# Anttwo/MACARONS

Measured on AMD Instinct MI355X. Metric: candidate-camera coverage-gain evals/sec (100k pts, 200 cams), higher is better.
Workload: dtype f32; 1 GPU; scorer: B=1 cloud x N=100000 points x C=200 cameras per GPU (BASELINE headline 100k pts / 200 cams), inputs resident in HBM; points=100000, cams_per_gpu=200, parallelism=camera-shard x1, streams=2

## Files before the change

macarons_amd/csrc/networks.hip:

```cpp
#include "nn_kernels.h"
#include "net_layout.h"
#include <cstdlib>
#include <algorithm>
#include <map>
#include <mutex>
#include <utility>

namespace mcr {

#ifdef MCR_DEV_LOCAL_PCT8
void launch_local_pct8(hipStream_t s, const float* offs, float* feat, int64_t ld_feat, int64_t S, const float* blob);
#define MCR_VARIANT8_OK(v) ((v) == 8)
#else
#define MCR_VARIANT8_OK(v) false
#endif
static int g_default_variant = []() {
    const char* e = getenv("MCR_LOCAL_PCT_VARIANT");
    const int v = e ? atoi(e) : 6;
    return (v == 1 || v == 5 || v == 6) ? v : 6;
}();
static thread_local int t_next_variant = 0;
static thread_local int t_variant = 0;
static thread_local int t_scope_depth = 0;
struct VariantScope {
// ... 454 lines not shown
    if (planes) {
        launch_linear_smallk_planes(s, {pts, 4}, l1.w, l1.b, ACT_GELU, h128, T, VIS_F, 4, 128);
        const float* b2 = w.b_l2p;
        const WPlanes W2 = weight_planes(s, w.p_l2, WSPLIT_INV, l2, VIS_F, VIS_F, VIS_F, ff, 128, 128, &b2);
        launch_linear3p(s, h128, W2, {b2, ACT_NONE}, {x, VIS_E}, T, 128, 128, np);
    } else {
        launch_linear(s, {pts, 4}, {l1.w, 4}, {l1.b, ACT_GELU}, {h, VIS_F}, T, VIS_F, 4, N);
        launch_linear(s, {h, VIS_F}, {l2.w, VIS_F}, {l2.b, ACT_NONE}, {x, VIS_E}, T, VIS_F, VIS_F, N);
    }
    launch_colmax_broadcast(s, x, VIS_E, x + VIS_F, VIS_E, B, (int)N, VIS_F, lengths, pts, 4, 4, x + 2 * VIS_F);
    for (int e = 0; e < 3; ++e) run_encoder(s, w.enc[e], x, h, qkv, ff, B, (int)N, VIS_E, 4, lengths);
    if (planes) {
        launch_layernorm_planes(s, {x, VIS_E}, w.ng, w.nb, hP.keep(np), T, VIS_E);
        _Float16* q = reinterpret_cast<_Float16*>(qkv);
        const WPlanes W1 = weight_planes(s, w.p_fc1, WSPLIT_INV, fc1, VIS_E, 192, VIS_E, q);
        const WPlanes W2 = weight_planes(s, w.p_fc2, WSPLIT_INV, fc2, VIS_E, 128, VIS_E, q + 2 * 192 * VIS_E);
        const WPlanes W3 = weight_planes(s, w.p_fc3, WSPLIT_INV, fc3, 128, 64, 128, q + 2 * (192 + 128) * VIS_E);
        const Planes fP = planes_over(ff, T, VIS_E);
        launch_linear3p(s, hP, W1, {fc1.b, ACT_GELU}, fP, T, 192, VIS_E, np);
        launch_split_to_planes(s, {view_harmonics, 64}, fP.cols(192).keep(np), T, 64);
        launch_linear3p(s, fP, W2, {fc2.b, ACT_GELU}, h128, T, 128, VIS_E, np);
        launch_linear3p(s, h128, W3, {fc3.b, ACT_NONE}, {out, 64}, T, 64, 128, np);
    } else {
        launch_layernorm(s, x, VIS_E, w.ng, w.nb, h, VIS_E, T, VIS_E);
        launch_linear(s, {h, VIS_E}, {fc1.w, VIS_E}, {fc1.b, ACT_GELU}, {ff, VIS_E}, T, 192, VIS_E, seq_route(N));
        launch_copy2d(s, view_harmonics, 64, ff + 192, VIS_E, T, 64);
        launch_linear(s, {ff, VIS_E}, {fc2.w, VIS_E}, {fc2.b, ACT_GELU}, {h, 128}, T, 128, VIS_E, seq_route(N));
        launch_linear(s, {h, 128}, {fc3.w, 128}, {fc3.b, ACT_NONE}, {out, 64}, T, 64, 128, N);
    }
    MCR_LAUNCH_CHECK("mcr_scone_vis_forward");
    return 0;
}

constexpr int OCC_CHUNK = 16384;
constexpr int FEAT = 1344;
constexpr size_t OCC_WS_SLACK = 8192 + 2 * 1024, OCC_RAGGED_WS_SLACK = 8192 + 1024;

struct OccHead {
    float *feat, *h1, *h2, *gfeat, *gbias;
    void* wplanes;
    HeadScratch planes() const { return HeadScratch{reinterpret_cast<_Float16*>(feat), reinterpret_cast<_Float16*>(h1), h2, wplanes}; }
};
static OccHead carve_occ_head(Arena& a, int64_t T, int64_t G) {
    OccHead w;
    w.feat = a.f(T * FEAT);
    w.h1 = a.f(T * 512);
    w.h2 = a.f(T * 256);
    w.gfeat = a.f(G * 512);
    w.gbias = a.f(G * 512);
    w.wplanes = a.bytes(linear3h_planes_bytes(512, 1344));
    return w;
}

struct OccSide { hipStream_t s = nullptr; hipEvent_t fork = nullptr, join = nullptr; };
static OccSide* occ_side(hipStream_t caller, int slot = 0) {
    static const bool on = []() { const char* e = getenv("MCR_OCC_OVERLAP"); return !(e && e[0] == '0'); }();
    if (!on) return nullptr;
    static std::mutex mu;
    static std::map<std::pair<std::pair<int, int>, hipStream_t>, OccSide> table;
    int dev = 0;
    if (hipGetDevice(&dev) != hipSuccess) return nullptr;
    std::lock_guard<std::mutex> lock(mu);
    OccSide& x = table[std::make_pair(std::make_pair(dev, slot), caller)];
    if (!x.s) {
        if (hipStreamCreateWithFlags(&x.s, hipStreamNonBlocking) != hipSuccess || hipEventCreateWithFlags(&x.fork, hipEventDisableTiming) != hipSuccess ||
            hipEventCreateWithFlags(&x.join, hipEventDisableTiming) != hipSuccess) {
            x.s = nullptr;
            return nullptr;
        }
    }
    return &x;
}
static hipStream_t fork_side(hipStream_t s, OccSide*& side) {
    if (side && hipEventRecord(side->fork, s) == hipSuccess && hipStreamWaitEvent(side->s, side->fork, 0) == hipSuccess) return side->s;
    side = nullptr;
    return s;
}
struct SideJoin {
    OccSide* side; hipStream_t s; bool recorded = false, joined = false;
    ~SideJoin() {
        if (!side || joined) return;
        if (!recorded) (void)hipEventRecord(side->join, side->s);
        (void)hipStreamWaitEvent(s, side->join, 0);
    }
};

static void run_global(hipStream_t gs, const OccW& w, const float* pc_global, int64_t G, int64_t Lg, const int* lens, const EncScratch& glob,
                       const OccHead& hd) {
    run_pct(gs, w.global, pc_global, hd.gfeat, 512, G, (int)Lg, 256, glob, lens);
    launch_linear(gs, {hd.gfeat, 512}, {w.lin1.w, 1856}, {nullptr, ACT_NONE}, {hd.gbias, 512}, G, 512, 512, 1);
}

static void head_linear(hipStream_t s, int which, Rows X, const LinW& lin, int64_t ldw, RowsOut Y, int64_t M, int N, int K, RowBias rb,
                        const void* const* head_planes, const float* head_inv_scales, void* wplanes) {
    const int variant = g_local_pct_variant;
    const int64_t ANY_M = (int64_t)1 << 40;
    const Rows W{lin.w, ldw};
    const Epilogue e{lin.b, ACT_GELU, {}, rb};
    if ((variant == 6 || variant == 7) && linear3h_applicable(X.p, X.ld, W.p, W.ld, ANY_M, N, K))
        launch_linear3h(s, X, head_weight_planes(s, which, lin, ldw, N, K, head_planes, head_inv_scales, wplanes), e, Y, M, N, K);
    else if (variant == 5 && linear3_applicable(X.p, X.ld, W.p, W.ld, ANY_M, N, K))
        launch_linear3(s, X, W, e, Y, M, N, K);
    else
        launch_linear(s, X, W, e, Y, M, N, K, 1);
}

static int run_occ_head(const char* who, hipStream_t s, const OccW& w, const float* x, const float* view_harmonics, int64_t T, const OccHead& hd,
                        int64_t rows_per_group, const int* row_group, const void* const* head_planes, const float* head_inv_scales, bool planes,
                        bool x_done, OccSide* side, SideJoin& side_join, int* range_flag, float* out) {
    bool join_failed = false;
    auto join = [&]() {
        if (side) {
            side_join.joined = true;
            join_failed = hipStreamWaitEvent(s, side->join, 0) != hipSuccess;
        }
    };
    if (planes)
        run_head_planes(s, x, view_harmonics, T, w.xe1, w.xe2, w.xe3, w.lin1, w.lin2, w.lin3, hd.gbias, rows_per_group, row_group, head_planes,
                        head_inv_scales, hd.planes(), out, join, x_done);
    else {
        launch_linear(s, {x, 3}, {w.xe1.w, 3}, {w.xe1.b, ACT_GELU}, {hd.h2, 128}, T, 128, 3, 1);
        head_linear(s, 0, {hd.h2, 128}, w.xe2, 128, {hd.h1, 256}, T, 256, 128, {}, head_planes, head_inv_scales, hd.wplanes);
        head_linear(s, 1, {hd.h1, 256}, w.xe3, 256, {hd.feat + 768, FEAT}, T, 512, 256, {}, head_planes, head_inv_scales, hd.wplanes);
        launch_copy2d(s, view_harmonics, 64, hd.feat + 1280, FEAT, T, 64);
        join();
        MCR_REQUIRE(!join_failed, "%s: side stream (join)", who);
        head_linear(s, 2, {hd.feat, FEAT}, {w.lin1.w + 512, w.lin1.b}, 1856, {hd.h1, 512}, T, 512, FEAT, {hd.gbias, rows_per_group, row_group},
                    head_planes, head_inv_scales, hd.wplanes);
        head_linear(s, 3, {hd.h1, 512}, w.lin2, 512, {hd.h2, 256}, T, 256, 512, {}, head_planes, head_inv_scales, hd.wplanes);
        launch_linear(s, {hd.h2, 256}, {w.lin3.w, 256}, {w.lin3.b, ACT_GELU}, {out, 1}, T, 1, 256, 1);
    }
    MCR_REQUIRE(!join_failed, "%s: side stream (join)", who);
    if (range_flag) launch_nonfinite_flag(s, out, T, range_flag);
    MCR_LAUNCH_CHECK(who);
    return 0;
}

struct OccLocal { float* offs; EncScratch pct; };
static OccLocal carve_occ_local(Arena& a, int64_t rows, bool layer_by_layer) {
    OccLocal w{};
    w.offs = a.f(rows * 16 * 3);
    if (layer_by_layer) w.pct = carve_enc(a, rows * 16, PCT_E);
    return w;
}
struct OccScratch {
    OccHead head;
    char *knn_q, *knn_c, *knn_park;
    size_t knn_c_bytes;
    EncScratch glob;
    Arena scratch;
};
static OccScratch carve_occ(Arena& a, int64_t B, int64_t Q, int64_t Lg) {
    OccScratch w;
    w.head = carve_occ_head(a, B * Q, B);
    w.knn_c_bytes = knn_grid_cloud_bytes(B, 16384);
    w.knn_q = (char*)a.bytes(knn_grid_query_bytes(B, Q));
    w.knn_c = (char*)a.bytes(3 * w.knn_c_bytes);
    w.knn_park = (char*)a.bytes(knn_grid_park_bytes());
    w.glob = carve_enc(a, B * Lg, PCT_E);
    w.scratch = a.rest();
    return w;
}
size_t mcr_scone_occ_workspace_bytes(int64_t B, int64_t Q, int64_t Lg) {
    const size_t local = std::max({measure(carve_occ_local, B * Q, false), measure(carve_occ_local, Q, false),
                                   measure(carve_occ_local, std::min<int64_t>(Q, OCC_CHUNK), true)});
    return measure(carve_occ, B, Q, Lg) + local + OCC_WS_SLACK;
}

int mcr_knn_points(const float* X, const float* pc, int64_t* idx, float* dists, float* pts, int64_t B, int64_t Q, int64_t M,
                   int k, int subtract_query, void* stream);

int mcr_scone_occ_forward_phase(const float* pc_global, int64_t Lg, const float* const* pc_scale, const int64_t* M_scale,
                                const float* x, const float* view_harmonics, float* out, int64_t B, int64_t Q,
                                const float* const* weights, int n_weights, const float* const* local_blobs,
                                const void* const* head_planes, const float* head_inv_scales, int* range_flag, void* workspace,
                                size_t workspace_bytes, int phase, void* stream) {
    const char* who = "mcr_scone_occ_forward";
    VariantScope variant_scope_;
    MCR_REQUIRE(phase >= 0 && phase <= 2, "mcr_scone_occ_forward: phase must be 0, 1 or 2");
    const bool early = phase != 2, late = phase != 1;
    MCR_REQUIRE(pc_scale && M_scale && x && weights && (!late || (pc_global && view_harmonics && out)), "mcr_scone_occ_forward: null pointer");
    MCR_REQUIRE(!head_planes || head_inv_scales, "mcr_scone_occ_forward: head_planes need head_inv_scales");
    if (check_table(who, OCC_TABLE, weights, n_weights, n_weights)) return 1;
    MCR_REQUIRE(B > 0 && Q > 0 && Lg > 0 && B <= 65535, "mcr_scone_occ_forward: bad problem size");
    MCR_REQUIRE(workspace && workspace_bytes >= mcr_scone_occ_workspace_bytes(B, Q, Lg), "mcr_scone_occ_forward: workspace too small");
    for (int i = 0; i < 3; ++i)
        MCR_REQUIRE((pc_scale[i] || (!late && i > 0)) && M_scale[i] >= 16, "mcr_scone_occ_forward: scale %d has %ld points (< k = 16)", i,
                    (long)M_scale[i]);
    hipStream_t s = (hipStream_t)stream;
    const OccW w = read_occ_table(weights, n_weights);
    Arena arena{(char*)workspace, workspace_bytes};
    const OccScratch ws = carve_occ(arena, B, Q, Lg);
    MCR_REQUIRE(arena.ok(), "mcr_scone_occ_forward: workspace overflow (global)");
    const OccHead& hd = ws.head;
    float* feat = hd.feat;

    OccSide* side = late ? occ_side(s) : nullptr;
    const hipStream_t gs = fork_side(s, side);
    SideJoin side_join{side, s};
    const bool fused_all = local_blobs && local_blobs[0] && local_blobs[1] && local_blobs[2];
    const int64_t qc = fused_all ? Q : std::min<int64_t>(Q, OCC_CHUNK);
    const bool planes = fused_all && fp16_planes_variant();
    const int64_t Tall = B * Q;
    const Planes featP = planes_over(hd.feat, Tall, FEAT);
    OccSide* xside = planes ? occ_side(s, 1) : nullptr;
    struct XJoin {
        OccSide* side; hipStream_t s; bool armed;
        bool wait() { if (!armed) return true; armed = false; return hipStreamWaitEvent(s, side->join, 0) == hipSuccess; }
        ~XJoin() { (void)wait(); }
    } x_join{xside, s, false};
    if (xside && early) {
        MCR_REQUIRE(hipEventRecord(xside->fork, s) == hipSuccess && hipStreamWaitEvent(xside->s, xside->fork, 0) == hipSuccess,
                    "mcr_scone_occ_forward: side stream (x embedding fork)");
        run_x_embedding_planes(xside->s, x, nullptr, B * Q, w.xe1, w.xe2, w.xe3, head_planes, head_inv_scales, hd.planes());
        MCR_REQUIRE(hipEventRecord(xside->join, xside->s) == hipSuccess, "mcr_scone_occ_forward: side stream (x embedding record)");
        x_join.armed = true;
    }
    if (late) {
        run_global(gs, w, pc_global, B, Lg, nullptr, ws.glob, hd);
        if (xside)
            launch_split_to_planes(gs, {view_harmonics, 64}, featP.cols(1280).keep(matrix_planes()), B * Q, 64);
    }
    if (side) {
        MCR_REQUIRE(hipEventRecord(side->join, side->s) == hipSuccess, "mcr_scone_occ_forward: side stream (record)");
        side_join.recorded = true;
    }
    const int* knn_qperm = nullptr;
    KnnGridCloud knn_clouds[3]{};
    int knn_slot[3] = {-1, -1, -1};
    if (qc == Q) {
        const float* g_pc[3]; int64_t g_M[3]; void* g_ws[3];
        int n_grid = 0;
        for (int sc = 0; sc < 3; ++sc)
            if (knn_grid_applicable(M_scale[sc], 16)) {
                g_pc[n_grid] = pc_scale[sc]; g_M[n_grid] = M_scale[sc]; g_ws[n_grid] = ws.knn_c + n_grid * ws.knn_c_bytes;
                knn_slot[sc] = n_grid++;
            }
        if (n_grid) {
            if (phase == 0) {
                knn_qperm = knn_grid_order_queries(s, x, B, Q, ws.knn_q, ws.knn_park);
                knn_grid_build_clouds(s, n_grid, g_pc, g_M, B, g_ws, knn_clouds);
            } else {
                const int first = early ? 0 : (knn_slot[0] >= 0 ? 1 : 0), count = early ? (knn_slot[0] >= 0 ? 1 : 0) : n_grid - first;
                OccSide* bside = early && count > 0 ? occ_side(s) : nullptr;
                const hipStream_t bs = fork_side(s, bside);
                knn_grid_build_clouds(bs, count, g_pc + first, g_M + first, B, g_ws + first, knn_clouds + first);
                const bool recorded = !bside || hipEventRecord(bside->join, bside->s) == hipSuccess;
                knn_qperm = knn_grid_order_queries(s, x, B, Q, ws.knn_q, ws.knn_park, early);
                const bool joined = !bside || hipStreamWaitEvent(s, bside->join, 0) == hipSuccess;
                MCR_REQUIRE(recorded && joined, "mcr_scone_occ_forward: side stream (cloud build)");
            }
            MCR_LAUNCH_CHECK("knn grid preparation");
        }
    }
    for (int sc = 0; sc < 3; ++sc) {
        if (sc == 0 ? !early : !late) continue;
        const bool grid_knn = knn_slot[sc] >= 0;
        const KnnGridCloud knn_cloud = grid_knn ? knn_clouds[knn_slot[sc]] : KnnGridCloud{};
        const bool fused = planes || (local_blobs && local_blobs[sc]);
        if (B > 1 && qc == Q && fused) {
            Arena a = ws.scratch;
            float* offs = carve_occ_local(a, Tall, false).offs;
            MCR_REQUIRE(a.ok(), "mcr_scone_occ_forward: workspace overflow (kNN)");
            if (grid_knn) {
                launch_knn16_grid(s, x, pc_scale[sc], M_scale[sc], knn_qperm, knn_cloud, 0, B, Q, nullptr, nullptr, offs, true, ws.knn_park, sc);
                MCR_LAUNCH_CHECK("knn_grid_kernel");
            } else if (int e = mcr_knn_points(x, pc_scale[sc], nullptr, nullptr, offs, B, Q, M_scale[sc], 16, 1, stream))
                return e;
            if (planes) run_local_pct(s, offs, nullptr, FEAT, Tall, local_blobs[sc], featP.cols(sc * 256));
            else run_local_pct(s, offs, feat + sc * 256, FEAT, Tall, local_blobs[sc]);
            continue;
        }
        for (int64_t q0 = 0; q0 < Q; q0 += qc) {
            const int64_t nq = std::min<int64_t>(qc, Q - q0);
            for (int64_t b = 0; b < B; ++b) {
                Arena a = ws.scratch;
                const OccLocal loc = carve_occ_local(a, nq, !fused);
                MCR_REQUIRE(a.ok(), fused ? "mcr_scone_occ_forward: workspace overflow (kNN)" : "mcr_scone_occ_forward: workspace overflow (local)");
                float* offs = loc.offs;
// ... 113 lines not shown
```

macarons_amd/nbv.py:

```python

import torch

from . import dist as mdist
from .utility import scone_utils as su


class ViewStateGrid:

    def __init__(self, device, degree=8, n_elev=7, n_azim=14):
        self.n_elev, self.n_azim = n_elev, n_azim
        self.base_harmonics, self.h_polar, self.h_azim = su.get_all_harmonics_under_degree(degree, n_elev, n_azim, device)


_side_streams = {}


def _harmonics_beside(scone_occ, pc, Xl, harmonics_of):
    dev = Xl.device
    main = torch.cuda.current_stream(dev)
    fork = torch.cuda.Event()
    fork.record(main)
    begun = scone_occ.forward_begin(pc, Xl)
    if begun is None:
        return begun, harmonics_of(Xl)
    side = _side_streams.get((dev.index, main.cuda_stream))
    if side is None:
        side = _side_streams[(dev.index, main.cuda_stream)] = torch.cuda.Stream(device=dev)
    side.wait_event(fork)
    with torch.cuda.stream(side):
        vh = harmonics_of(Xl)
    main.wait_stream(side)
    vh.record_stream(main)
    return begun, vh


def _guarded(impl, scone_occ, range_guard, group, draws, device, scone_vis=None):
    from . import ops
    capturing = torch.cuda.is_current_stream_capturing()
    prev = scone_occ.range_guard
    guard = range_guard and prev != "off" and ops.current_variant() in (6, 7)
    scone_occ.range_guard = "defer" if (guard or prev != "off") else "off"
    vis_prev = None
    if scone_vis is not None and hasattr(scone_vis, "range_guard"):
        vis_prev = (scone_vis.range_guard, scone_vis._range_flag)
        scone_vis.range_guard = scone_occ.range_guard
    try:
        flagged = scone_occ.range_guard != "off" and ops.current_variant() in (6, 7)
        scone_occ.clear_range_flag(device if flagged else None)
        if vis_prev is not None:
            scone_vis._range_flag = scone_occ.range_flag()
        kw = draws() if (guard and not capturing) else {}
        out = impl(**kw)
        flag = scone_occ.range_flag() if ops.current_variant() in (6, 7) else None
        out["range_flag"] = flag
        if guard and not capturing:
            xch = mdist.exchange_on(group)
            if xch:
                flag = mdist.all_reduce_max(flag, group)
            if not xch and "record" in out:
                both = out["record"].cpu()
            else:
                both = torch.cat((flag.to(out["nbv_idx"].device).view(-1).to(torch.float64), out["nbv_idx"].view(-1).to(torch.float64),
                                  out["max_gain"].view(-1).to(torch.float64))).cpu()
            n_dec = out["nbv_idx"].numel()
            out["host"] = {"nbv_idx": both[1:1 + n_dec].to(torch.int64), "max_gain": both[1 + n_dec:].to(torch.float32)}
            if int(both[0]):
                with ops.variant(5):
                    out = impl(**kw)
                out["range_flag"], out["fallback_variant"] = None, 5
                out.pop("host", None)
    finally:
        scone_occ.range_guard = prev
        if vis_prev is not None:
            scone_vis.range_guard, scone_vis._range_flag = vis_prev
    return out


def nbv_step(scone_occ, scone_vis, pc, X, X_view, X_cam, grid, seq_len=2048, min_occ=0.1,
             max_points_per_pass=300000, true_monte_carlo_sampling=True, occ_perms=None, samples=None, group=None,
             view_proj=None, filter_tol=0.01, return_samples=False, range_guard=True):
    if X.shape[0] > 1:
        if view_proj is not None or max_points_per_pass < X.shape[1] * X.shape[0]:
            raise NotImplementedError("nbv_step: the proxy filter / multi-chunk occupancy pass are single-cloud options")
# ... 8 lines not shown
        if fixed["samples"] is None:
            fixed["samples"] = torch.rand(seq_len, 1, device=X.device)
        return {}

    def impl():
        return _nbv_step(scone_occ, scone_vis, pc, X, X_view, X_cam, grid, seq_len, min_occ, max_points_per_pass,
                         true_monte_carlo_sampling, fixed["occ_perms"], fixed["samples"], group, view_proj, filter_tol, return_samples)
    if mdist.group_world_rank(group)[0] > 1:
        draws = lambda: {}
    return _guarded(impl, scone_occ, range_guard, group, draws, X.device, scone_vis)


def nbv_step_one_rank_of(world, scone_occ, scone_vis, pc, X, X_view, X_cam, grid, occ_perms, samples, rank=0, seq_len=2048, min_occ=0.1):
    return _guarded(lambda: _nbv_step(scone_occ, scone_vis, pc, X, X_view, X_cam, grid, seq_len, min_occ, occ_perms=occ_perms, samples=samples,
                                      _emulate=(rank, world)), scone_occ, False, None, lambda: {}, X.device, scone_vis)


def _nbv_step(scone_occ, scone_vis, pc, X, X_view, X_cam, grid, seq_len=2048, min_occ=0.1,
              max_points_per_pass=300000, true_monte_carlo_sampling=True, occ_perms=None, samples=None, group=None,
              view_proj=None, filter_tol=0.01, return_samples=False, _emulate=None):
    world, rank = mdist.group_world_rank(group)
    sharded = mdist.exchange_on(group)
    gather_rows, gather_best = mdist.allgather_rows, mdist.allgather_best
    if _emulate is not None:
        rank, world = _emulate
        sharded = True
        gather_rows = lambda t, n, g_=None: t.repeat(-(-n // max(t.shape[0], 1)), 1)[:n].contiguous()
        def gather_best(g_, c0_, grp=None):
            b_ = torch.max(g_, dim=1)
            return b_.values, b_.indices + c0_
    dev = X.device
    if view_proj is not None:
        X = su.filter_proxy_points(view_proj, X[0], pc.reshape(-1, 3), filter_tol=filter_tol)[0][None]
    Q = X.shape[1]
    if Q == 0:
        raise ValueError("nbv_step: no proxy point left to score (the proxy filter removed every point)")
    with torch.no_grad():
        q0, q1 = mdist.shard_range(Q, rank, world)
        Xl = X[:, q0:q1].contiguous()
        if sharded and _emulate is None and (occ_perms is None or samples is None):
            draw_perms, draw_u = occ_perms is None, samples is None
            if draw_perms:
                occ_perms = [p.to(dev) for p in scone_occ.draw_perms(pc.shape[1])]
            if draw_u:
                samples = torch.rand(seq_len, 1, device=dev)
            got_p, got_u = mdist.broadcast_draws(occ_perms if draw_perms else [], samples if draw_u else None, 0, group)
            if draw_perms:
                occ_perms = got_p
            if draw_u:
                samples = got_u
        if q1 > q0:
            harmonics_of = lambda pts: su.compute_view_harmonics(su.compute_view_state(pts, X_view, grid.n_elev, grid.n_azim),
                                                                 grid.base_harmonics, grid.h_polar, grid.h_azim, grid.n_elev, grid.n_azim)
            begun, vh_l = _harmonics_beside(scone_occ, pc, Xl, harmonics_of) if occ_perms is not None else (None, harmonics_of(Xl))
            if occ_perms is not None:
                occ_l = scone_occ(pc, Xl, vh_l, perms=occ_perms, begun=begun).view(-1, 1)
            else:
                occ_l = su.compute_occupancy_probability(scone_occ, pc, Xl, vh_l, max_points_per_pass=max_points_per_pass).view(-1, 1)
        else:
            vh_l = torch.zeros(1, 0, grid.base_harmonics.shape[0], dtype=torch.float32, device=dev)
            occ_l = torch.zeros(0, 1, dtype=torch.float32, device=dev)
        if sharded:
            occ = gather_rows(occ_l, Q, group)
            vh = None
        else:
            occ, vh = occ_l, vh_l[0]
        if samples is None:
            samples = torch.rand(seq_len, 1, device=dev)
        if vh is not None:
            proxy_points, vh_s, sample_idx, n_unique = su.sample_proxy_points(X[0], occ, vh, n_sample=seq_len, min_occ=min_occ,
                                                                              samples=samples, padded=True)
        else:
            from . import ops
            proxy_points, _, sample_idx, _, n_unique = ops.sample_proxy(X[0].contiguous(), occ.reshape(-1), None, samples.reshape(-1),
                                                                        min_occ, padded=True)
            vs_s = su.compute_view_state(proxy_points[None, :, :3].contiguous(), X_view, grid.n_elev, grid.n_azim)
            vh_s = su.compute_view_harmonics(vs_s, grid.base_harmonics, grid.h_polar, grid.h_azim, grid.n_elev, grid.n_azim)[0]
        sampled = (proxy_points, sample_idx)
        harm = scone_vis(proxy_points[None], view_harmonics=vh_s[None], lengths=n_unique)
        if true_monte_carlo_sampling:
            proxy_points, harm = proxy_points[sample_idx][None].contiguous(), harm[0][sample_idx][None].contiguous()
        else:
            k = int(n_unique)
            proxy_points, harm = proxy_points[:k][None].contiguous(), harm[:, :k].contiguous()
        C = X_cam.shape[0]
        c0, c1 = mdist.shard_range(C, rank, world)
        if c1 > c0:
            gains = scone_vis.compute_coverage_gain(proxy_points, harm, X_cam[c0:c1].contiguous().view(1, -1, 3))
        else:
            gains = torch.zeros(1, 0, dtype=torch.float32, device=dev)
        record = None
        if sharded:
            empty = n_unique.view(1, 1) < 1
            gains = torch.where(empty, torch.full_like(gains, float("nan")), gains)
            max_gain, nbv_idx = gather_best(gains, c0, group)
            nbv_idx = torch.where(empty.view(-1), torch.full_like(nbv_idx, -1), nbv_idx)
        else:
            from . import ops
            flag = scone_occ.range_flag() if scone_occ.range_guard != "off" else None
            max_gain, nbv_idx, record = ops.nbv_decide(gains, n_unique.view(-1), flag)
    out = {"gains": gains[0], "cam_range": (c0, c1), "nbv_idx": nbv_idx, "max_gain": max_gain, "occ": occ,
           "n_unique": n_unique}
    if record is not None:
        out["record"] = record
    if return_samples:
        out["proxy_points"], out["sample_idx"] = sampled
    return out
# ... 6 lines not shown
    return perms, samples


def nbv_step_batch(scone_occ, scone_vis, pc, X, X_view, X_cam, grid, seq_len=2048, min_occ=0.1, true_monte_carlo_sampling=True,
                   occ_perms=None, samples=None, group=None, return_samples=False, range_guard=True):
    fixed = dict(occ_perms=occ_perms, samples=samples)
    xch = mdist.exchange_on(group)

    def draws():
        if not xch and (fixed["occ_perms"] is None or fixed["samples"] is None):
            dp, du = draw_batch(scone_occ, X.shape[0], pc.shape[1], seq_len, X.device)
            fixed["occ_perms"] = dp if fixed["occ_perms"] is None else fixed["occ_perms"]
            fixed["samples"] = du if fixed["samples"] is None else fixed["samples"]
        return {}

    def impl():
        return _nbv_step_batch(scone_occ, scone_vis, pc, X, X_view, X_cam, grid, seq_len, min_occ, true_monte_carlo_sampling,
                               fixed["occ_perms"], fixed["samples"], group, return_samples)
    return _guarded(impl, scone_occ, range_guard, group, draws, X.device, scone_vis)


def _nbv_step_batch(scone_occ, scone_vis, pc, X, X_view, X_cam, grid, seq_len=2048, min_occ=0.1, true_monte_carlo_sampling=True,
                    occ_perms=None, samples=None, group=None, return_samples=False):
    from . import ops
    world, rank = mdist.group_world_rank(group)
    dev = X.device
    B, Q, M, C = X.shape[0], X.shape[1], pc.shape[1], X_cam.shape[-2]
    if pc.shape[0] != B:
        raise ValueError("nbv_step_batch: pc and X must hold the same number of clouds")
    xch = mdist.exchange_on(group)
    by_cloud = xch and B >= world
    with torch.no_grad():
        if occ_perms is None or samples is None:
            dp, du = draw_batch(scone_occ, B, M, seq_len, dev)
            if xch:
                got_p, got_u = mdist.broadcast_draws(dp if occ_perms is None else [], du if samples is None else None, 0, group)
                dp, du = (got_p if occ_perms is None else dp), (got_u if samples is None else du)
            occ_perms = dp if occ_perms is None else occ_perms
            samples = du if samples is None else samples
        samples = samples.reshape(B, seq_len).to(dev)
        occ_perms = [p.to(dev) for p in occ_perms]
        b0, b1 = mdist.shard_range(B, rank, world) if by_cloud else (0, B)
        q0, q1 = (0, Q) if (by_cloud or not xch) else mdist.shard_range(Q, rank, world)
        c0, c1 = (0, C) if (by_cloud or not xch) else mdist.shard_range(C, rank, world)
        Bl = b1 - b0
        pc_l, X_b = pc[b0:b1].contiguous(), X[b0:b1].contiguous()
        Xv_l = X_view[b0:b1].contiguous() if X_view.dim() == 3 else X_view
        perms_l = [p[b0:b1] if p.dim() == 2 else p for p in occ_perms]
        u_l = samples[b0:b1].contiguous()
        vs_of = lambda pts: su.compute_view_harmonics(su.compute_view_state(pts, Xv_l, grid.n_elev, grid.n_azim), grid.base_harmonics,
                                                      grid.h_polar, grid.h_azim, grid.n_elev, grid.n_azim)
        if q1 > q0:
            Xl = X_b[:, q0:q1].contiguous()
            begun, vh_l = _harmonics_beside(scone_occ, pc_l, Xl, vs_of)
            occ_l = scone_occ(pc_l, Xl, vh_l, perms=perms_l, begun=begun).view(Bl, q1 - q0)
        else:
            vh_l, occ_l = None, torch.zeros(Bl, 0, dtype=torch.float32, device=dev)
        if q1 - q0 < Q:
            occ = mdist.allgather_rows(occ_l.t().contiguous(), Q, group).t().contiguous()
            vh_l = None
        else:
            occ = occ_l
        res, resh, inv, uniq, nu, _ = ops.sample_proxy_batched(X_b, occ, vh_l, u_l, min_occ)
        if resh is None:
            resh = vs_of(res[..., :3].contiguous())
        harm = scone_vis(res, view_harmonics=resh, lengths=nu)
        if true_monte_carlo_sampling:
            pts_s = torch.gather(res, 1, inv[..., None].expand(-1, -1, 4))
            harm_s = torch.gather(harm, 1, inv[..., None].expand(-1, -1, 64))
        else:
            raise NotImplementedError("nbv_step_batch scores the Monte-Carlo multiset (true_monte_carlo_sampling=True)")
        cams = X_cam[b0:b1] if X_cam.dim() == 3 else X_cam[None].expand(Bl, -1, -1)
        cams = cams[:, c0:c1].contiguous()
        gains = scone_vis.compute_coverage_gain(pts_s, harm_s, cams) if c1 > c0 else torch.zeros(Bl, 0, dtype=torch.float32, device=dev)
        record = None
        if not xch:
            flag = scone_occ.range_flag() if scone_occ.range_guard != "off" else None
            max_gain, nbv_idx, record = ops.nbv_decide(gains, nu.view(-1), flag)
        else:
            gains = torch.where(nu.view(-1, 1) < 1, torch.full_like(gains, float("nan")), gains)
            if by_cloud:
                rec = mdist.allgather_rows(ops.best_record(gains, 0), B, group)
                max_gain, nbv_idx = rec[:, 0].contiguous(), rec[:, 1].to(torch.int64)
                nbv_idx = torch.where(torch.isnan(max_gain), torch.full_like(nbv_idx, -1), nbv_idx)
            else:
                max_gain, nbv_idx = mdist.allgather_best(gains, c0, group)
                nbv_idx = torch.where(nu < 1, torch.full_like(nbv_idx, -1), nbv_idx)
    out = {"gains": gains, "cloud_range": (b0, b1), "cam_range": (c0, c1), "max_gain": max_gain, "nbv_idx": nbv_idx,
           "occ": occ.view(Bl, Q, 1), "n_unique": nu}
    if record is not None:
        out["record"] = record
    if return_samples:
        out["proxy_points"], out["sample_idx"] = res, inv
    return out


class GraphedNbvStep:

    def __init__(self, scone_occ, scone_vis, pc, X, X_view, X_cam, grid, seq_len=2048, min_occ=0.1, warmup=2, one_rank_of=None):
        self.one_rank_of = one_rank_of
        if torch.distributed.is_available() and torch.distributed.is_initialized() and torch.distributed.get_world_size() > 1:
            raise RuntimeError("GraphedNbvStep captures the single-GPU step; use nbv_step under torchrun")
        self.occ, self.vis, self.grid, self.seq_len, self.min_occ = scone_occ, scone_vis, grid, seq_len, min_occ
        dev = X.device
        self._in = {"pc": pc.clone(), "X": X.clone(), "X_view": X_view.clone(), "X_cam": X_cam.clone(),
                    "samples": torch.empty(seq_len, 1, device=dev),
                    "perms": [p.to(dev) for p in scone_occ.draw_perms(pc.shape[1])]}
# ... 35 lines not shown
```

macarons_amd/networks/SconeOcc.py:

```python
import numpy as np
import os
import torch
import torch.nn.functional as F
from torch import nn

from .. import autograd as A
from .. import ops, _lib
from .Attention import (Embedding, Encoder, FeedForward, MultiHeadSelfAttention, attention, knn_gather,
                        _f32c, _inference_only)
from ..utility.utils import get_knn_points
from .packing import encoder_weight_planes, padded_weight_planes, weight_planes, RangeGuard, BlobCache, HeadPlaneCache, TableCache, param_key, invalidate as _invalidate_key, freeze as _freeze_key


class XEmbedding(nn.Module):

    def __init__(self, x_dim, x_embedding_dim, dropout=None, gelu=True):
        super().__init__()
        if not gelu or dropout is not None:
            raise NotImplementedError("HIP path implements the GELU / no-dropout configuration")
        self.linear1 = nn.Linear(x_dim, x_embedding_dim // 4)
        self.linear2 = nn.Linear(x_embedding_dim // 4, x_embedding_dim // 2)
        self.linear3 = nn.Linear(x_embedding_dim // 2, x_embedding_dim)
        self.non_linear1, self.non_linear2, self.non_linear3 = nn.GELU(), nn.GELU(), nn.GELU()
        self.dropout = None
# ... 328 lines not shown
            d = ops.h2d(flat, torch.int64, dev)
            cut, o = [], 0
            for n in (J * Lg, n1, n2, J + 1, J + 1, J):
                cut.append(d[o:o + n]); o += n
            ia = {"g_idx": cut[0], "idx1": cut[1], "idx2": cut[2], "off1": cut[3], "off2": cut[4], "g_len": cut[5].to(torch.int32)}
            self.last_ragged_perms = ia
            pc_global = pc[ia["g_idx"]].view(J, Lg, 3)
            pc1 = pc[ia["idx1"]]
            pc2 = pc1[ia["idx2"]]
            g_len_d, d_off1, d_off2 = ia["g_len"], ia["off1"], ia["off2"]

        def run(v, flag, redo_phase1, out_):
            if redo_phase1:
                phase1(v)
            blobs, head, table = state[v] if v in state else caches(v)
            return ops.scone_occ_forward_ragged(pc_global, g_len_d, [pc, pc1, pc2], [d_off0, d_off1, d_off2], x, view_harmonics,
                                                d_row_job, d_blocks, table, blobs, head, flag, phase=2, out=out_, arena=h["arena"])
        if differentiable and A.needs_grad(self, x, view_harmonics):
            params, slots = self._grad_slots()
            sz = [self.scale_sizes(int(m)) for m in cloud_sizes]
            return A.SconeOccRaggedFunction.apply(
                lambda: run(variant, None, ops.scone_occ_epoch(dev, h["arena"]) != h["epoch1"], None), self.weight_table, slots,
                [[s_[i] for s_ in sz] for i in range(self.n_scale)], h["query_sizes"], pc_global, g_len_d, [pc, pc1, pc2], d_row_job,
                x, view_harmonics, *params)
        flag = None
        guard = self._effective_guard()
        if variant in (6, 7) and guard != "off":
            if self._range_flag is None or self._range_flag.device != dev:
                self._range_flag = torch.zeros(1, dtype=torch.int32, device=dev)
            elif guard in ("sync", "async"):
                self._range_flag.zero_()
            flag = self._range_flag
        with torch.no_grad():
            res = run(variant, flag, ops.scone_occ_epoch(dev, h["arena"]) != h["epoch1"], out)
            if flag is not None and guard == "sync" and int(flag):
                with ops.variant(5):
                    res = run(5, None, True, out)
            elif flag is not None and guard == "async":
                self._post_range_check(flag)
        return res

    def scale_sizes(self, full_seq_len):
        ds, sizes = self.ds_factor(full_seq_len), [full_seq_len]
        for _ in range(self.n_scale - 1):
            sizes.append(sizes[-1] // ds)
        return sizes

    def _images(self, variant):
        key = param_key(self, self._key_cache)
        blobs = [c.get(t, variant, key) for c, t in zip(self._blob_caches, self.local_transformers)] if self.fused_local else None
        head = self._head_cache.get(self, key) if variant in (6, 7) else None
        return self._table_cache.get(self, self.weight_table_with_planes, key), blobs, head

    def forward_begin(self, pc, x):
        if not self._is_default_arch() or not self.fused_local or A.needs_grad(self, pc, x):
            return None
        variant = ops.current_variant()
        pc0, x_ = pc.contiguous(), x.contiguous()
        sizes = self.scale_sizes(pc.shape[1])
        if min(sizes) < self.k_for_knn:
            return None
        with torch.no_grad():
            table, blobs, head = self._images(variant)
            ops.scone_occ_forward(None, [pc0, None, None], x_, None, table, blobs, head, None, phase=1, M_scale=sizes, Lg=self.seq_len)
        return {"pc": pc0, "x": x_, "variant": variant, "sizes": sizes, "src": (pc, x), "epoch": ops.scone_occ_epoch(pc0.device, "scone_occ")}

    def forward(self, pc, x, view_harmonics, mask=None, verbose=False, perms=None, begun=None):
        if mask is not None:
            raise NotImplementedError("SconeOcc.forward(mask=...): upstream applies the same mask to sequences of 2048 and of 16 tokens")
        if not self._is_default_arch():
            raise NotImplementedError("the fused MI355X SconeOcc forward implements the reference's default architecture")
        n_clouds, full_seq_len = pc.shape[0], pc.shape[1]
        n_sample = x.shape[1]
        if perms is None:
            perms = self.draw_perms(full_seq_len)
        dev = pc.device
        L = _lib.lib()
        if self._effective_guard() == "async" and (self._range_pending or self._full_range):
            self.check_range()
        if self._full_range and ops.current_variant() in (6, 7):
            with ops.variant(5):
                return self.forward(pc, x, view_harmonics, mask, verbose, perms, None)
        variant = ops.current_variant()
        sizes = self.scale_sizes(full_seq_len)
        if begun is not None and not (begun["src"][0] is pc and begun["src"][1] is x and begun["variant"] == variant
                                      and begun["sizes"] == sizes and [p_.shape[-1] for p_ in perms] == [self.seq_len] + sizes[1:]
                                      and begun["epoch"] == ops.scone_occ_epoch(dev, "scone_occ")):
            begun = None
        pc_global = self._take(pc, perms[0])
        scales = [begun["pc"] if begun is not None else pc.contiguous()]
        for p in perms[1:]:
            scales.append(self._take(scales[-1], p))
        phase = 0
        if begun is not None:
            phase, x = 2, begun["x"]

        def run(variant, pc_global, scales, x_, vh_, flag, phase=0):
            table, blobs, head = self._images(variant)
            return ops.scone_occ_forward(pc_global, scales, x_, vh_, table, blobs, head, flag, phase=phase)

        flag = None
        guard = self._effective_guard()
        if variant in (6, 7) and guard != "off":
            if self._range_flag is None or self._range_flag.device != dev:
                self._range_flag = torch.zeros(1, dtype=torch.int32, device=dev)
            elif guard in ("sync", "async"):
                self._range_flag.zero_()
            flag = self._range_flag
        if A.needs_grad(self, pc, x, view_harmonics) and A.scone_occ_backward_mode() == "hip" and not pc.requires_grad:
            params, slots = self._grad_slots()
            res = A.SconeOccFunction.apply(lambda g_, sc_, x_, vh_: run(variant, g_, sc_, x_, vh_, None), self.weight_table, slots,
                                           self.k_for_knn, pc_global, scales, x, view_harmonics, *params)
        elif A.needs_grad(self, pc, x, view_harmonics):
            pidx = [p.to(dev) for p in perms]

            def clouds(pc_):
                sc = [pc_.contiguous()]
                for p in pidx[1:]:
                    sc.append(self._take(sc[-1], p))
                return self._take(pc_, pidx[0]), sc

            def hip(pc_, x_, vh_):
                g, sc = clouds(pc_)
                return run(variant, g, sc, x_, vh_, None)

            def composite(pc_, x_, vh_):
                g, sc = clouds(pc_)
                with torch.no_grad():
                    idx = [ops.knn_points(x_.detach().contiguous(), s_.detach(), self.k_for_knn)[2] for s_ in sc]
                return A.scone_occ(self, g, sc, x_, vh_, idx)
            res = A.with_torch_backward(hip, composite, (pc, x, view_harmonics), self)
        else:
            res = run(variant, pc_global, scales, x, view_harmonics, flag, phase)
            if flag is not None and guard == "sync" and int(flag):
                with ops.variant(5):
                    res = run(5, pc_global, scales, x, view_harmonics, None)
            elif flag is not None and guard == "async":
                self._post_range_check(flag)
        return res.view(n_clouds, n_sample, self.output_dim)
```

macarons_amd/ops.py:

```python
import os
import ctypes
import torch
import numpy as np

from ._lib import lib, check, MacaronsHipError, c_i64, c_int, c_size, c_vp, c_f32
from .utility.host import limit_host_threads

limit_host_threads()


def _stream():
    return c_vp(torch.cuda.current_stream().cuda_stream)


def _req(t, name, dtype=torch.float32):
    if not isinstance(t, torch.Tensor):
        raise TypeError(f"{name} must be a torch.Tensor")
    if not t.is_cuda:
        raise MacaronsHipError(f"{name} must live on a HIP device (got {t.device}); "
                               "the MI355X hot path has no CPU fallback")
    if t.dtype != dtype:
        raise TypeError(f"{name} must be {dtype} (got {t.dtype})")
    return t.contiguous()

# ... 591 lines not shown
    if acc and (not d_x.is_contiguous() or d_x.dtype != torch.float32 or d_x.shape != x.shape):
        raise ValueError("d_x must be a contiguous float32 tensor shaped like x")
    dx = d_x if acc else torch.empty_like(x2)
    need_g, need_b = bool(need[1]), bool(need[2])
    dg = torch.empty((E,), dtype=torch.float32, device=x.device) if need_g else None
    db = torch.empty((E,), dtype=torch.float32, device=x.device) if need_b else None
    ptr = lambda t: _p(t) if t is not None else c_vp(None)
    L_ = lib()
    ws = _workspace(x.device, int(L_.mcr_layernorm_backward_workspace_bytes(c_i64(M), c_int(E))))
    with torch.cuda.device(x.device):
        check(L_.mcr_layernorm_backward(_p(x2), c_i64(E), _p(weight), _p(d_y.reshape(M, E)), c_i64(E), c_i64(M), c_int(E), _p(dx), c_i64(E),
                                        c_int(int(acc)), ptr(dg), ptr(db), _p(ws), c_size(ws.numel()), _stream()), "mcr_layernorm_backward")
    return dx.reshape(*lead, E), dg, db


def colmax_backward(x, d_bcast, d_x, lens=None):
    x, d_bcast = _req(x, "x"), _req(d_bcast, "d_bcast")
    S, L, E = x.shape
    if d_bcast.shape != x.shape or not d_x.is_contiguous() or d_x.shape != x.shape or d_x.dtype != torch.float32:
        raise ValueError("colmax_backward: x, d_bcast and d_x must all be [S,L,E] (d_x contiguous float32)")
    if lens is not None:
        lens = _req(lens, "lens", torch.int32).reshape(-1)
        if lens.numel() != S:
            raise ValueError(f"lens must hold one length per sequence ({S}), got {lens.numel()}")
    with torch.cuda.device(x.device):
        check(lib().mcr_colmax_backward(_p(x), c_i64(E), _p(d_bcast), c_i64(E), _p(d_x), c_i64(E), c_i64(S), c_i64(L), c_int(E),
                                        _p(lens) if lens is not None else c_vp(0), _stream()), "mcr_colmax_backward")
    return d_x


def nonfinite_flag_(x, flag):
    x = _req(x, "x")
    if x.numel():
        with torch.cuda.device(x.device):
            check(lib().mcr_nonfinite_flag(_p(x), c_i64(x.numel()), _p(_req(flag, "flag", torch.int32)), _stream()), "mcr_nonfinite_flag")
    return flag


def local_pct_forward(offsets, blob):
    offsets, blob = _req(offsets, "offsets"), _req(blob, "blob")
    S = offsets.shape[0]
    if tuple(offsets.shape[1:]) != (16, 3):
        raise ValueError("offsets must be [S,16,3]")
    out = torch.empty((S, 256), dtype=torch.float32, device=offsets.device)
    with torch.cuda.device(offsets.device):
        check(_net(lib()).mcr_local_pct_forward(_p(offsets), _p(out), c_i64(256), c_i64(S), _p(blob), _stream()),
              "mcr_local_pct_forward")
    return out


def scone_occ_forward(pc_global, pc_scales, x, view_harmonics, weights, local_blobs=None, head_planes=None, range_flag=None, phase=0,
                      M_scale=None, Lg=None, out=None):
    late = phase != 1
    x = _req(x, "x")
    B, Q = x.shape[0], x.shape[1]
    if late:
        pc_global, view_harmonics = _req(pc_global, "pc_global"), _req(view_harmonics, "view_harmonics")
        pc_scales = [_req(p, "pc_scale") for p in pc_scales]
        Lg = pc_global.shape[1]
        M_scale = [p.shape[1] for p in pc_scales]
        if pc_global.shape[0] != B or len(pc_scales) != 3 or x.shape != (B, Q, 3) or view_harmonics.shape != (B, Q, 64):
            raise ValueError("SconeOcc HIP path needs 3 scales, x [B,Q,3] and view_harmonics [B,Q,64]")
    else:
        pc_scales = [_req(pc_scales[0], "pc_scale"), None, None]
        if x.shape != (B, Q, 3) or M_scale is None or len(M_scale) != 3 or Lg is None or pc_scales[0].shape[1] != M_scale[0]:
            raise ValueError("SconeOcc phase 1 needs x [B,Q,3], the whole cloud, the three scale sizes and Lg")
    L_ = lib()
    if late and out is None:
        out = torch.empty((B, Q, 1), dtype=torch.float32, device=x.device)
    nb = L_.mcr_scone_occ_workspace_bytes(c_i64(B), c_i64(Q), c_i64(Lg))
    ws = _workspace(x.device, nb, "scone_occ")
    _bump_epoch(x.device, "scone_occ")
    tab = _ptr_table(weights)
    sc_ptrs = (ctypes.c_void_p * 3)(*[p.data_ptr() if p is not None else None for p in pc_scales])
    sc_m = (ctypes.c_int64 * 3)(*[int(m) for m in M_scale])
    blobs = (ctypes.c_void_p * 3)(*[_req(b, "local_blob").data_ptr() for b in local_blobs]) if local_blobs else None
    with torch.cuda.device(x.device):
        check(_net(L_).mcr_scone_occ_forward_phase(_p(pc_global) if late else c_vp(0), c_i64(Lg), sc_ptrs, sc_m, _p(x),
                                             _p(view_harmonics) if late else c_vp(0), _p(out) if late else c_vp(0), c_i64(B),
                                             c_i64(Q), tab, c_int(_n_weights(weights)), blobs,
                                             head_planes[1] if head_planes is not None else None,
                                             head_planes[2] if head_planes is not None else None,
                                             _p(_req(range_flag, "range_flag", torch.int32)) if range_flag is not None else c_vp(0),
                                             _p(ws), c_size(ws.numel()), c_int(int(phase)), _stream()),
              "mcr_scone_occ_forward")
    return out


def scone_occ_forward_ragged(pc_global, global_len, pc_scales, scale_offsets, x, view_harmonics, row_job, knn_blocks, weights,
                             local_blobs, head_planes=None, range_flag=None, phase=0, Lg=None, out=None, arena="scone_occ_ragged"):
    x, view_harmonics = _req(x, "x"), _req(view_harmonics, "view_harmonics")
    row_job = _req(row_job, "row_job", torch.int32)
    knn_blocks = _req(knn_blocks, "knn_blocks", torch.int32)
    late = phase != 1
    pc_scales = [_req(p, "pc_scale") for p in (pc_scales if late else [pc_scales[0]] * 3)]
    scale_offsets = [_req(o, "scale_offsets", torch.int64) for o in (scale_offsets if late else [scale_offsets[0]] * 3)]
    J = scale_offsets[0].numel() - 1
    if late:
        pc_global, global_len = _req(pc_global, "pc_global"), _req(global_len, "global_len", torch.int32)
        Lg = pc_global.shape[1]
        if pc_global.shape[0] != J or global_len.numel() != J:
            raise ValueError("scone_occ_forward_ragged: pc_global [J,Lg,3], global_len [J]")
    T = x.shape[0]
    if x.shape != (T, 3) or view_harmonics.shape != (T, 64) or row_job.numel() != T:
        raise ValueError("scone_occ_forward_ragged: x [T,3], view_harmonics [T,64], row_job [T]")
    if any(o.numel() != J + 1 for o in scale_offsets) or knn_blocks.dim() != 2 or knn_blocks.shape[1] != 4:
        raise ValueError("scone_occ_forward_ragged: scale_offsets must be [J+1], knn_blocks [n_blocks,4]")
    L_ = lib()
    if late and out is None:
        out = torch.empty((T, 1), dtype=torch.float32, device=x.device)
    ws = _workspace(x.device, L_.mcr_scone_occ_ragged_workspace_bytes(c_i64(J), c_i64(T), c_i64(Lg)), arena)
    _bump_epoch(x.device, arena)
    sc_ptrs = (ctypes.c_void_p * 3)(*[p.data_ptr() for p in pc_scales])
    off_ptrs = (ctypes.c_void_p * 3)(*[o.data_ptr() for o in scale_offsets])
    blobs = (ctypes.c_void_p * 3)(*[_req(b, "local_blob").data_ptr() for b in local_blobs])
    with torch.cuda.device(x.device):
        check(_net(L_).mcr_scone_occ_forward_ragged_phase(_p(pc_global) if late else c_vp(0), _p(global_len) if late else c_vp(0), c_i64(Lg), sc_ptrs,
                                                    off_ptrs, _p(x), _p(view_harmonics), _p(row_job), _p(knn_blocks), c_i64(knn_blocks.shape[0]),
                                                    _p(out) if late else c_vp(0), c_i64(J), c_i64(T),
                                                    _ptr_table(weights), c_int(_n_weights(weights)), blobs,
                                                    head_planes[1] if head_planes is not None else None,
                                                    head_planes[2] if head_planes is not None else None,
                                                    _p(_req(range_flag, "range_flag", torch.int32)) if range_flag is not None else c_vp(0),
                                                    _p(ws), c_size(ws.numel()), c_int(int(phase)), _stream()), "mcr_scone_occ_forward_ragged")
    return out


def view_state(pts, X_view, n_elev, n_azim):
    pts, X_view = _req(pts, "pts"), _req(X_view, "X_view")
    B, Q, d = pts.shape
    out = torch.empty((B, Q, n_elev * n_azim), dtype=torch.float32, device=pts.device)
# ... 1048 lines not shown
```

Baseline: 4.873 million evals/s.

## Run all three kNN searches and global encoder early on a side stream

When the point-cloud permutations are known ahead of time, phase 1 now gathers the global and scale clouds and runs all three kNN searches, with the scale-1/2 searches and the global encoder on a side stream. Phase 3 then only runs the local PCTs and the head. The Python side launches the view-harmonics computation on a side stream before forward_begin when perms are given. The aim is to overlap the kNN, global encoder and harmonics work with main-stream work, and to move more of the front-end out of the serialized late phase. In exchange it adds two extra offset buffers and a second park buffer to the workspace, more events, and more complex cross-stream synchronization.

```diff
diff --git a/macarons_amd/csrc/networks.hip b/macarons_amd/csrc/networks.hip
--- a/macarons_amd/csrc/networks.hip
+++ b/macarons_amd/csrc/networks.hip
@@ -530,7 +530,7 @@
     return w;
 }
 
-struct OccSide { hipStream_t s = nullptr; hipEvent_t fork = nullptr, join = nullptr; };
+struct OccSide { hipStream_t s = nullptr; hipEvent_t fork = nullptr, join = nullptr, ready = nullptr, go = nullptr, found = nullptr; };
 static OccSide* occ_side(hipStream_t caller, int slot = 0) {
     static const bool on = []() { const char* e = getenv("MCR_OCC_OVERLAP"); return !(e && e[0] == '0'); }();
     if (!on) return nullptr;
@@ -542,7 +542,9 @@
     OccSide& x = table[std::make_pair(std::make_pair(dev, slot), caller)];
     if (!x.s) {
         if (hipStreamCreateWithFlags(&x.s, hipStreamNonBlocking) != hipSuccess || hipEventCreateWithFlags(&x.fork, hipEventDisableTiming) != hipSuccess ||
-            hipEventCreateWithFlags(&x.join, hipEventDisableTiming) != hipSuccess) {
+            hipEventCreateWithFlags(&x.join, hipEventDisableTiming) != hipSuccess ||
+            hipEventCreateWithFlags(&x.ready, hipEventDisableTiming) != hipSuccess || hipEventCreateWithFlags(&x.go, hipEventDisableTiming) != hipSuccess ||
+            hipEventCreateWithFlags(&x.found, hipEventDisableTiming) != hipSuccess) {
             x.s = nullptr;
             return nullptr;
         }
@@ -623,8 +625,9 @@
 }
 struct OccScratch {
     OccHead head;
-    char *knn_q, *knn_c, *knn_park;
+    char *knn_q, *knn_c, *knn_park, *knn_park_side;
     size_t knn_c_bytes;
+    float* offs_side[2];
     EncScratch glob;
     Arena scratch;
 };
@@ -635,6 +638,8 @@
     w.knn_q = (char*)a.bytes(knn_grid_query_bytes(B, Q));
     w.knn_c = (char*)a.bytes(3 * w.knn_c_bytes);
     w.knn_park = (char*)a.bytes(knn_grid_park_bytes());
+    w.knn_park_side = (char*)a.bytes(knn_grid_park_bytes());
+    for (float*& o : w.offs_side) o = a.f(B * Q * 16 * 3);
     w.glob = carve_enc(a, B * Lg, PCT_E);
     w.scratch = a.rest();
     return w;
@@ -655,8 +660,9 @@
                                 size_t workspace_bytes, int phase, void* stream) {
     const char* who = "mcr_scone_occ_forward";
     VariantScope variant_scope_;
-    MCR_REQUIRE(phase >= 0 && phase <= 2, "mcr_scone_occ_forward: phase must be 0, 1 or 2");
-    const bool early = phase != 2, late = phase != 1;
+    MCR_REQUIRE(phase >= 0 && phase <= 3, "mcr_scone_occ_forward: phase must be 0, 1, 2 or 3");
+    const bool early = phase < 2, late = phase != 1;
+    const bool rich = phase == 1 && pc_global && pc_scale && pc_scale[1] && pc_scale[2];
     MCR_REQUIRE(pc_scale && M_scale && x && weights && (!late || (pc_global && view_harmonics && out)), "mcr_scone_occ_forward: null pointer");
     MCR_REQUIRE(!head_planes || head_inv_scales, "mcr_scone_occ_forward: head_planes need head_inv_scales");
     if (check_table(who, OCC_TABLE, weights, n_weights, n_weights)) return 1;
@@ -673,36 +679,108 @@
     const OccHead& hd = ws.head;
     float* feat = hd.feat;
 
-    OccSide* side = late ? occ_side(s) : nullptr;
-    const hipStream_t gs = fork_side(s, side);
-    SideJoin side_join{side, s};
     const bool fused_all = local_blobs && local_blobs[0] && local_blobs[1] && local_blobs[2];
     const int64_t qc = fused_all ? Q : std::min<int64_t>(Q, OCC_CHUNK);
     const bool planes = fused_all && fp16_planes_variant();
     const int64_t Tall = B * Q;
     const Planes featP = planes_over(hd.feat, Tall, FEAT);
     OccSide* xside = planes ? occ_side(s, 1) : nullptr;
+    const bool front = fused_all && (phase == 0 || rich || phase == 3) && occ_side(s);
+    const bool front_now = front && phase != 3;
+    if (phase == 3 && !front) phase = 2;
+    OccSide* side = (front ? (front_now || xside) : late) ? occ_side(s) : nullptr;
+    const hipStream_t gs = fork_side(s, side);
+    SideJoin side_join{side, s};
+    struct FoundJoin {
+        OccSide* side; hipStream_t s; bool armed;
+        bool wait() { if (!armed) return true; armed = false; return hipStreamWaitEvent(s, side->found, 0) == hipSuccess; }
+        ~FoundJoin() { (void)wait(); }
+    } found_join{side, s, false};
     struct XJoin {
         OccSide* side; hipStream_t s; bool armed;
         bool wait() { if (!armed) return true; armed = false; return hipStreamWaitEvent(s, side->join, 0) == hipSuccess; }
         ~XJoin() { (void)wait(); }
     } x_join{xside, s, false};
-    if (xside && early) {
+    auto queue_x_embedding = [&]() {
+        if (!(xside && early)) return true;
+        run_x_embedding_planes(xside->s, x, nullptr, B * Q, w.xe1, w.xe2, w.xe3, head_planes, head_inv_scales, hd.planes());
+        if (hipEventRecord(xside->join, xside->s) != hipSuccess) return false;
+        return x_join.armed = true;
+    };
+    if (xside && early)
         MCR_REQUIRE(hipEventRecord(xside->fork, s) == hipSuccess && hipStreamWaitEvent(xside->s, xside->fork, 0) == hipSuccess,
                     "mcr_scone_occ_forward: side stream (x embedding fork)");
-        run_x_embedding_planes(xside->s, x, nullptr, B * Q, w.xe1, w.xe2, w.xe3, head_planes, head_inv_scales, hd.planes());
-        MCR_REQUIRE(hipEventRecord(xside->join, xside->s) == hipSuccess, "mcr_scone_occ_forward: side stream (x embedding record)");
-        x_join.armed = true;
-    }
-    if (late) {
-        run_global(gs, w, pc_global, B, Lg, nullptr, ws.glob, hd);
-        if (xside)
+    if (!front_now) MCR_REQUIRE(queue_x_embedding(), "mcr_scone_occ_forward: side stream (x embedding record)");
+    auto queue_global = [&]() {
+        if (front ? front_now : late) run_global(gs, w, pc_global, B, Lg, nullptr, ws.glob, hd);
+        if (late && xside)
             launch_split_to_planes(gs, {view_harmonics, 64}, featP.cols(1280).keep(matrix_planes()), B * Q, 64);
-    }
-    if (side) {
-        MCR_REQUIRE(hipEventRecord(side->join, side->s) == hipSuccess, "mcr_scone_occ_forward: side stream (record)");
-        side_join.recorded = true;
-    }
+        if (side) {
+            if (hipEventRecord(side->join, side->s) != hipSuccess) return false;
+            side_join.recorded = true;
+        }
+        return true;
+    };
+    if (front) {
+        Arena a = ws.scratch;
+        float* const offs[3] = {carve_occ_local(a, Tall, false).offs, ws.offs_side[0], ws.offs_side[1]};
+        MCR_REQUIRE(a.ok(), "mcr_scone_occ_forward: workspace overflow (kNN)");
+        auto local = [&](int sc) {
+            if (planes) run_local_pct(s, offs[sc], nullptr, FEAT, Tall, local_blobs[sc], featP.cols(sc * 256));
+            else run_local_pct(s, offs[sc], feat + sc * 256, FEAT, Tall, local_blobs[sc]);
+        };
+        if (front_now) {
+            const float* g_pc[3]; int64_t g_M[3]; void* g_ws[3];
+            KnnGridCloud clouds[3]{};
+            int slot[3] = {-1, -1, -1}, n_grid = 0;
+            for (int sc = 0; sc < 3; ++sc)
+                if (knn_grid_applicable(M_scale[sc], 16)) {
+                    g_pc[n_grid] = pc_scale[sc]; g_M[n_grid] = M_scale[sc]; g_ws[n_grid] = ws.knn_c + n_grid * ws.knn_c_bytes;
+                    slot[sc] = n_grid++;
+                }
+            const int* qperm = nullptr;
+            if (n_grid) {
+                bool ok = hipMemsetAsync(ws.knn_park_side, 0, 256, gs) == hipSuccess;
+                knn_grid_build_clouds(gs, n_grid, g_pc, g_M, B, g_ws, clouds);
+                ok = ok && (!side || hipEventRecord(side->ready, gs) == hipSuccess);
+                qperm = knn_grid_order_queries(s, x, B, Q, ws.knn_q, ws.knn_park);
+                ok = ok && (!side || (hipStreamWaitEvent(s, side->ready, 0) == hipSuccess && hipEventRecord(side->go, s) == hipSuccess &&
+                                      hipStreamWaitEvent(gs, side->go, 0) == hipSuccess));
+                MCR_REQUIRE(ok, "mcr_scone_occ_forward: side stream (cloud builds / query order)");
+                MCR_LAUNCH_CHECK("knn grid preparation");
+            }
+            for (int sc = 0; sc < 3; ++sc) {
+                const hipStream_t ss = sc == 0 ? s : gs;
+                if (slot[sc] >= 0) {
+                    launch_knn16_grid(ss, x, pc_scale[sc], M_scale[sc], qperm, clouds[slot[sc]], 0, B, Q, nullptr, nullptr, offs[sc], true,
+                                      sc == 0 ? ws.knn_park : ws.knn_park_side, sc);
+                    MCR_LAUNCH_CHECK("knn_grid_kernel");
+                } else if (int e = mcr_knn_points(x, pc_scale[sc], nullptr, nullptr, offs[sc], B, Q, M_scale[sc], 16, 1, ss))
+                    return e;
+            }
+            if (side) {
+                MCR_REQUIRE(hipEventRecord(side->found, gs) == hipSuccess, "mcr_scone_occ_forward: side stream (searches, record)");
+                found_join.armed = true;
+            }
+            MCR_REQUIRE(queue_x_embedding(), "mcr_scone_occ_forward: side stream (x embedding record)");
+            MCR_REQUIRE(queue_global(), "mcr_scone_occ_forward: side stream (record)");
+            local(0);
+            MCR_REQUIRE(found_join.wait(), "mcr_scone_occ_forward: side stream (searches, join)");
+        } else
+            MCR_REQUIRE(queue_global(), "mcr_scone_occ_forward: side stream (record)");
+        if (late) {
+            local(1);
+            local(2);
+        }
+        MCR_REQUIRE(x_join.wait(), "mcr_scone_occ_forward: side stream (x embedding join)");
+        if (!late) {
+            MCR_LAUNCH_CHECK("mcr_scone_occ_forward (phase 1)");
+            return 0;
+        }
+        return run_occ_head(who, s, w, x, view_harmonics, Tall, hd, Q, nullptr, head_planes, head_inv_scales, planes, xside != nullptr,
+                            side, side_join, range_flag, out);
+    }
+    MCR_REQUIRE(queue_global(), "mcr_scone_occ_forward: side stream (record)");
     const int* knn_qperm = nullptr;
     KnnGridCloud knn_clouds[3]{};
     int knn_slot[3] = {-1, -1, -1};
diff --git a/macarons_amd/nbv.py b/macarons_amd/nbv.py
--- a/macarons_amd/nbv.py
+++ b/macarons_amd/nbv.py
@@ -15,20 +15,27 @@
 _side_streams = {}
 
 
-def _harmonics_beside(scone_occ, pc, Xl, harmonics_of):
+def _harmonics_beside(scone_occ, pc, Xl, harmonics_of, perms=None):
     dev = Xl.device
     main = torch.cuda.current_stream(dev)
     fork = torch.cuda.Event()
     fork.record(main)
-    begun = scone_occ.forward_begin(pc, Xl)
-    if begun is None:
-        return begun, harmonics_of(Xl)
-    side = _side_streams.get((dev.index, main.cuda_stream))
-    if side is None:
-        side = _side_streams[(dev.index, main.cuda_stream)] = torch.cuda.Stream(device=dev)
-    side.wait_event(fork)
-    with torch.cuda.stream(side):
-        vh = harmonics_of(Xl)
+
+    def beside():
+        side = _side_streams.get((dev.index, main.cuda_stream))
+        if side is None:
+            side = _side_streams[(dev.index, main.cuda_stream)] = torch.cuda.Stream(device=dev)
+        side.wait_event(fork)
+        with torch.cuda.stream(side):
+            return side, harmonics_of(Xl)
+    if perms is not None:
+        side, vh = beside()
+        begun = scone_occ.forward_begin(pc, Xl, perms)
+    else:
+        begun = scone_occ.forward_begin(pc, Xl)
+        if begun is None:
+            return begun, harmonics_of(Xl)
+        side, vh = beside()
     main.wait_stream(side)
     vh.record_stream(main)
     return begun, vh
@@ -143,7 +150,7 @@
         if q1 > q0:
             harmonics_of = lambda pts: su.compute_view_harmonics(su.compute_view_state(pts, X_view, grid.n_elev, grid.n_azim),
                                                                  grid.base_harmonics, grid.h_polar, grid.h_azim, grid.n_elev, grid.n_azim)
-            begun, vh_l = _harmonics_beside(scone_occ, pc, Xl, harmonics_of) if occ_perms is not None else (None, harmonics_of(Xl))
+            begun, vh_l = _harmonics_beside(scone_occ, pc, Xl, harmonics_of, occ_perms) if occ_perms is not None else (None, harmonics_of(Xl))
             if occ_perms is not None:
                 occ_l = scone_occ(pc, Xl, vh_l, perms=occ_perms, begun=begun).view(-1, 1)
             else:
@@ -256,7 +263,7 @@
                                                       grid.h_polar, grid.h_azim, grid.n_elev, grid.n_azim)
         if q1 > q0:
             Xl = X_b[:, q0:q1].contiguous()
-            begun, vh_l = _harmonics_beside(scone_occ, pc_l, Xl, vs_of)
+            begun, vh_l = _harmonics_beside(scone_occ, pc_l, Xl, vs_of, perms_l)
             occ_l = scone_occ(pc_l, Xl, vh_l, perms=perms_l, begun=begun).view(Bl, q1 - q0)
         else:
             vh_l, occ_l = None, torch.zeros(Bl, 0, dtype=torch.float32, device=dev)
diff --git a/macarons_amd/networks/SconeOcc.py b/macarons_amd/networks/SconeOcc.py
--- a/macarons_amd/networks/SconeOcc.py
+++ b/macarons_amd/networks/SconeOcc.py
@@ -404,7 +404,7 @@
         head = self._head_cache.get(self, key) if variant in (6, 7) else None
         return self._table_cache.get(self, self.weight_table_with_planes, key), blobs, head
 
-    def forward_begin(self, pc, x):
+    def forward_begin(self, pc, x, perms=None):
         if not self._is_default_arch() or not self.fused_local or A.needs_grad(self, pc, x):
             return None
         variant = ops.current_variant()
@@ -412,10 +412,20 @@
         sizes = self.scale_sizes(pc.shape[1])
         if min(sizes) < self.k_for_knn:
             return None
+        if perms is not None and (len(perms) != 3 or [p_.shape[-1] for p_ in perms] != [self.seq_len] + sizes[1:]):
+            perms = None
         with torch.no_grad():
             table, blobs, head = self._images(variant)
-            ops.scone_occ_forward(None, [pc0, None, None], x_, None, table, blobs, head, None, phase=1, M_scale=sizes, Lg=self.seq_len)
-        return {"pc": pc0, "x": x_, "variant": variant, "sizes": sizes, "src": (pc, x), "epoch": ops.scone_occ_epoch(pc0.device, "scone_occ")}
+            pc_global, scales = None, [pc0, None, None]
+            if perms is not None:
+                pc_global = self._take(pc, perms[0])
+                scales = [pc0, self._take(pc0, perms[1])]
+                scales.append(self._take(scales[1], perms[2]))
+            ops.scone_occ_forward(pc_global, scales, x_, None, table, blobs, head, None, phase=1, M_scale=sizes, Lg=self.seq_len)
+        h = {"pc": pc0, "x": x_, "variant": variant, "sizes": sizes, "src": (pc, x), "epoch": ops.scone_occ_epoch(pc0.device, "scone_occ")}
+        if perms is not None:
+            h["perms"], h["pc_global"], h["scales"] = tuple(perms), pc_global, scales
+        return h
 
     def forward(self, pc, x, view_harmonics, mask=None, verbose=False, perms=None, begun=None):
         if mask is not None:
@@ -439,13 +449,18 @@
                                       and begun["sizes"] == sizes and [p_.shape[-1] for p_ in perms] == [self.seq_len] + sizes[1:]
                                       and begun["epoch"] == ops.scone_occ_epoch(dev, "scone_occ")):
             begun = None
-        pc_global = self._take(pc, perms[0])
-        scales = [begun["pc"] if begun is not None else pc.contiguous()]
-        for p in perms[1:]:
-            scales.append(self._take(scales[-1], p))
+        if begun is not None and "perms" in begun and not (len(perms) == 3 and all(a is b for a, b in zip(begun["perms"], perms))):
+            begun = None
+        if begun is not None and "perms" in begun:
+            pc_global, scales = begun["pc_global"], begun["scales"]
+        else:
+            pc_global = self._take(pc, perms[0])
+            scales = [begun["pc"] if begun is not None else pc.contiguous()]
+            for p in perms[1:]:
+                scales.append(self._take(scales[-1], p))
         phase = 0
         if begun is not None:
-            phase, x = 2, begun["x"]
+            phase, x = (3 if "perms" in begun else 2), begun["x"]
 
         def run(variant, pc_global, scales, x_, vh_, flag, phase=0):
             table, blobs, head = self._images(variant)
diff --git a/macarons_amd/ops.py b/macarons_amd/ops.py
--- a/macarons_amd/ops.py
+++ b/macarons_amd/ops.py
@@ -667,9 +667,17 @@
 def scone_occ_forward(pc_global, pc_scales, x, view_harmonics, weights, local_blobs=None, head_planes=None, range_flag=None, phase=0,
                       M_scale=None, Lg=None, out=None):
     late = phase != 1
+    rich = phase == 1 and pc_global is not None and pc_scales[1] is not None and pc_scales[2] is not None
     x = _req(x, "x")
     B, Q = x.shape[0], x.shape[1]
-    if late:
+    if rich:
+        pc_global = _req(pc_global, "pc_global")
+        pc_scales = [_req(p, "pc_scale") for p in pc_scales]
+        Lg = pc_global.shape[1]
+        M_scale = [p.shape[1] for p in pc_scales]
+        if pc_global.shape[0] != B or len(pc_scales) != 3 or x.shape != (B, Q, 3) or any(p.shape[0] != B for p in pc_scales):
+            raise ValueError("SconeOcc phase 1 with the draws needs pc_global [B,Lg,3], 3 scales [B,M_i,3] and x [B,Q,3]")
+    elif late:
         pc_global, view_harmonics = _req(pc_global, "pc_global"), _req(view_harmonics, "view_harmonics")
         pc_scales = [_req(p, "pc_scale") for p in pc_scales]
         Lg = pc_global.shape[1]
@@ -691,7 +699,7 @@
     sc_m = (ctypes.c_int64 * 3)(*[int(m) for m in M_scale])
     blobs = (ctypes.c_void_p * 3)(*[_req(b, "local_blob").data_ptr() for b in local_blobs]) if local_blobs else None
     with torch.cuda.device(x.device):
-        check(_net(L_).mcr_scone_occ_forward_phase(_p(pc_global) if late else c_vp(0), c_i64(Lg), sc_ptrs, sc_m, _p(x),
+        check(_net(L_).mcr_scone_occ_forward_phase(_p(pc_global) if (late or rich) else c_vp(0), c_i64(Lg), sc_ptrs, sc_m, _p(x),
                                              _p(view_harmonics) if late else c_vp(0), _p(out) if late else c_vp(0), c_i64(B),
                                              c_i64(Q), tab, c_int(_n_weights(weights)), blobs,
                                              head_planes[1] if head_planes is not None else None,
```

Result: no change. 4.883 million evals/s (median of 3 runs) (+0.2%).
